# epifluidlab/FinaleToolkit

Hardware: AMD Instinct MI355X
Metric: genomic windows/sec (coverage+WPS+DELFI) at 30x WGS (higher is better)
Workload: dtype int32/int64

## Files before the change

finaletoolkit_amd/csrc/ftk_textparse.hip:

```cpp
#include <hip/hip_runtime.h>

#include <algorithm>

#include "ftk_textparse.h"

namespace ftk {
namespace {

constexpr int kT = 256;
constexpr int kB = 16;
static_assert(kT * kB == kTextBlockBytes, "block geometry");

struct Range {
    const uint8_t* text;
    size_t n;
    unsigned lead;
};
__device__ __forceinline__ Range range_of(const uint8_t* text, size_t n, const TextSummary* ind) {
    if (!ind) return {text, n, 0u};
    const unsigned off = ind->text_off, lead = off & 15u;
    return {text + (off - lead), ind->text_len ? (size_t)ind->text_len + lead : 0, lead};
}

__device__ __forceinline__ unsigned nl_mask16(const uint8_t* __restrict__ text, size_t off, size_t n, uint4& v) {
    unsigned m = 0;
    if (off + kB <= n) {
        v = *reinterpret_cast<const uint4*>(text + off);
    } else {
        unsigned w[4] = {0u, 0u, 0u, 0u};
        for (int j = 0; j < kB && off + j < n; ++j) w[j >> 2] |= (unsigned)text[off + j] << (8 * (j & 3));
        v = make_uint4(w[0], w[1], w[2], w[3]);
    }
    const unsigned w[4] = {v.x, v.y, v.z, v.w};
#pragma unroll
    for (int k = 0; k < 4; ++k)
#pragma unroll
        for (int j = 0; j < 4; ++j)
            if (((w[k] >> (8 * j)) & 0xffu) == (unsigned)'\n') m |= 1u << (4 * k + j);
    if (off + kB > n) m &= n > off ? (1u << (n - off)) - 1u : 0u;
    return m;
}

__device__ __forceinline__ unsigned wave_incl_scan(unsigned v, int lane) {
#pragma unroll
    for (int d = 1; d < 64; d <<= 1) {
        const unsigned t = __shfl_up(v, d, 64);
        if (lane >= d) v += t;
    }
    return v;
}

constexpr unsigned long long kAgg = 1ull << 32, kIncl = 2ull << 32;
__device__ __forceinline__ unsigned long long st_load(const unsigned long long* p) {
    return __hip_atomic_load(p, __ATOMIC_RELAXED, __HIP_MEMORY_SCOPE_AGENT);
}
__device__ __forceinline__ void st_store(unsigned long long* p, unsigned long long v) {
    __hip_atomic_store(p, v, __ATOMIC_RELAXED, __HIP_MEMORY_SCOPE_AGENT);
}

struct GlobalText {
    const uint8_t* __restrict__ p;
    __device__ __forceinline__ uint8_t operator[](uint32_t i) const { return p[i]; }
};
struct LdsText {
    const uint8_t* p;
    uint32_t base;
    __device__ __forceinline__ uint8_t operator[](uint32_t i) const { return p[i - base]; }
};

template <typename Text>
__device__ __forceinline__ bool dev_digits(const Text& t, uint32_t& p, uint32_t e, uint8_t term, unsigned long long& v) {
    const uint32_t s = p;
    unsigned long long x = 0;
    while (p < e) {
        const unsigned d = (unsigned)t[p] - (unsigned)'0';
        if (d > 9) break;
        x = x * 10 + d;
        ++p;
    }
    if (p == s || p - s > 10 || p >= e || t[p] != term) return false;
    ++p;
    v = x;
    return true;
}

template <typename Text>
__device__ __forceinline__ bool parse_row(const Text& t, size_t i, uint32_t b, uint32_t e, uint32_t pb, bool last,
                                          size_t max_lines, int bed6, int32_t* __restrict__ o_start, int32_t* __restrict__ o_end,
                                          uint8_t* __restrict__ o_mapq, uint8_t* __restrict__ o_strand,
                                          TextSummary* __restrict__ sum, int indirect) {
    uint32_t p = b;
    while (p < e && t[p] != '\t') ++p;
    const uint32_t name_len = p - b;
    unsigned long long fs = 0, fe = 0, mq = 0;
    uint8_t strand = 0;
    bool ok = name_len > 0 && p < e && t[b] != '#';
    if (ok) {
        ++p;
        ok = dev_digits(t, p, e, '\t', fs) && dev_digits(t, p, e, '\t', fe);
    }
    if (ok && bed6) {
        while (p < e && t[p] != '\t') ++p;
        ok = p < e;
        ++p;
    }
    if (ok) ok = dev_digits(t, p, e, '\t', mq);
    if (ok) {
        ok = p < e;
        if (ok) {
            strand = t[p];
            ok = strand != '\t' && strand != '\r';
            ++p;
            if (p < e && t[p] == '\r') ++p;
            ok = ok && p == e;
        }
    }
    ok = ok && fs <= 0x7fffffffull && fe <= 0x7fffffffull;
    if (ok && i < max_lines) {
        o_start[i] = (int32_t)fs;
        o_end[i] = (int32_t)fe;
        o_mapq[i] = (uint8_t)(mq < 255 ? mq : 255);
        o_strand[i] = strand == '+' ? 1 : 0;
        bool new_run = i == 0;
        if (!new_run) {
            const uint32_t pe = b - 1;
            new_run = pb + name_len >= pe || t[pb + name_len] != '\t';
            for (uint32_t k = 0; !new_run && k < name_len; ++k) new_run = t[pb + k] != t[b + k];
        }
        if (new_run) {
            const unsigned slot = atomicAdd(&sum->n_runs, 1u);
            if (slot < (unsigned)kTextMaxRuns) {
                sum->run_line[slot] = (unsigned)i;
                sum->run_off[slot] = b;
            }
            if (indirect) {
                if (slot < (unsigned)kTextNamedRuns && name_len < (uint32_t)kTextNameBytes) {
                    for (uint32_t k = 0; k < name_len; ++k) sum->run_name[slot][k] = t[b + k];
                    sum->run_name[slot][name_len] = 0;
                } else {
                    sum->name_overflow = 1;
                }
            }
        }
    }
    if (!ok && last) sum->last_line_bad = 1;
    return ok;
}

template <typename Text>
__device__ __forceinline__ uint32_t line_start_before(const Text& t, uint32_t from, uint32_t lead) {
    uint32_t p = from;
    while (p > lead && t[p - 1] != '\n') --p;
    return p;
}

constexpr int kHalo = 256;
constexpr int kMaxLinesPerBlock = 512;
__global__ __launch_bounds__(kT) void lines_rows_kernel(const uint8_t* __restrict__ text_, size_t n_,
                                                         unsigned long long* __restrict__ state, unsigned n_max_blocks,
                                                         size_t max_lines, int bed6, int32_t* __restrict__ o_start,
                                                         int32_t* __restrict__ o_end, uint8_t* __restrict__ o_mapq,
                                                         uint8_t* __restrict__ o_strand, TextSummary* __restrict__ sum,
                                                         int indirect) {
    __shared__ unsigned s_bid, s_base, s_first, s_prev;
    __shared__ unsigned wave_tot[kT / 64];
    __shared__ unsigned short nlpos[kMaxLinesPerBlock];
    __shared__ __align__(16) uint8_t s_text[kHalo + kTextBlockBytes];
    const int tid = threadIdx.x, lane = tid & 63, wv = tid >> 6;
    if (tid == 0) s_bid = atomicAdd(reinterpret_cast<unsigned*>(state + n_max_blocks), 1u);
    __syncthreads();
    const unsigned bid = s_bid;
    const Range R = range_of(text_, n_, indirect ? sum : nullptr);
    const uint8_t* __restrict__ text = R.text;
    const size_t n = R.n;
    const unsigned n_blocks = (unsigned)((n + kTextBlockBytes - 1) / kTextBlockBytes);
    if (bid >= n_blocks) {
        if (bid == 0 && tid == 0) sum->n_lines = 0;
        return;
    }
    const size_t blk_off = (size_t)bid * kTextBlockBytes;
    const size_t off = blk_off + (size_t)tid * kB;
    uint4 mine = make_uint4(0u, 0u, 0u, 0u);
    unsigned m = off < n ? nl_mask16(text, off, n, mine) : 0;
    *reinterpret_cast<uint4*>(&s_text[kHalo + tid * kB]) = mine;
    if (tid < kHalo / kB && bid > 0)
        *reinterpret_cast<uint4*>(&s_text[tid * kB]) = *reinterpret_cast<const uint4*>(text + blk_off - kHalo + (size_t)tid * kB);
    if (off == 0) m &= ~0u << R.lead;
    const unsigned c = __popc(m);
    const unsigned incl = wave_incl_scan(c, lane);
    if (lane == 63) wave_tot[wv] = incl;
    __syncthreads();
    unsigned before = 0, total = 0;
#pragma unroll
    for (int k = 0; k < kT / 64; ++k) {
        if (k < wv) before += wave_tot[k];
        total += wave_tot[k];
    }
    {
        unsigned idx = before + incl - c;
        while (m) {
            const int j = __ffs(m) - 1;
            m &= m - 1;
            if (idx < (unsigned)kMaxLinesPerBlock) nlpos[idx] = (unsigned short)(tid * kB + j);
            ++idx;
        }
    }
    if (wv == 0) {
        unsigned base = 0;
        if (bid > 0) {
            if (lane == 0) st_store(state + bid, kAgg | total);
            int j = (int)bid - 1;
            for (;;) {
                const int idx = j - lane;
                unsigned long long v = kIncl;
                if (idx >= 0)
                    do v = st_load(state + idx);
                    while ((v >> 32) == 0ull);
                const unsigned long long done = __ballot((v >> 32) == 2ull);
                const int stop = done ? __ffsll(done) - 1 : 63;
                unsigned part = lane <= stop ? (unsigned)v : 0u;
#pragma unroll
                for (int d = 32; d > 0; d >>= 1) part += __shfl_down(part, d, 64);
                base += (unsigned)__shfl(part, 0, 64);
                if (done) break;
                j -= 64;
            }
        }
        if (lane == 0) {
            st_store(state + bid, kIncl | (unsigned long long)(base + total));
            s_base = base;
            if (bid == n_blocks - 1) {
                sum->n_lines = (unsigned long long)base + total;
                if ((size_t)base + total > max_lines) sum->overflow = 1;
            }
        }
    }
    __syncthreads();
    if (total == 0) return;
    if (total > (unsigned)kMaxLinesPerBlock) {
        if (tid == 0) sum->overflow = 1;
        return;
    }
    const uint32_t lds_lo = bid > 0 ? (uint32_t)blk_off - (uint32_t)kHalo : 0u;
    const LdsText LT{s_text, (uint32_t)blk_off - (uint32_t)kHalo};
    const GlobalText GT{text};
    if (wv == 0) {
        const uint32_t e0 = (uint32_t)blk_off + nlpos[0];
        const uint32_t span = e0 - max(R.lead, lds_lo);
        const bool all_seen = lds_lo <= R.lead;
        const bool v0 = (uint32_t)lane < span, v1 = (uint32_t)lane + 64u < span;
        const unsigned long long m0 = __ballot(v0 && LT[e0 - 1u - (uint32_t)lane] == '\n');
        const unsigned long long m1 = __ballot(v1 && LT[e0 - 65u - (uint32_t)lane] == '\n');
        if (lane == 0) {
            const uint32_t seen = min(span, 128u);
            uint32_t f, pv;
            const int k1 = m0 ? __ffsll(m0) - 1 : (m1 ? 64 + __ffsll(m1) - 1 : -1);
            if (k1 >= 0) f = e0 - (uint32_t)k1;
            else f = (all_seen && span <= 128u) ? R.lead : line_start_before(GT, e0 - seen, R.lead);
            if (f == R.lead) {
                pv = f;
            } else {
                int k2 = -1;
                if (k1 >= 0) {
                    const unsigned long long r0 = k1 < 63 ? m0 & (~0ull << (k1 + 1)) : 0ull;
                    const unsigned long long r1 = k1 < 64 ? m1 : (k1 < 127 ? m1 & (~0ull << (k1 - 63)) : 0ull);
                    k2 = r0 ? __ffsll(r0) - 1 : (r1 ? 64 + __ffsll(r1) - 1 : -1);
                }
                if (k2 >= 0) pv = e0 - (uint32_t)k2;
                else if (k1 >= 0 && all_seen && span <= 128u) pv = R.lead;
                else pv = line_start_before(GT, k1 >= 0 ? e0 - seen : f - 1u, R.lead);
            }
            s_first = f;
            s_prev = pv;
        }
    }
    __syncthreads();
    const unsigned base = s_base;
    const uint32_t last_e = (uint32_t)(n - 1);
    for (unsigned k0 = 0; k0 < total; k0 += kT) {
        const unsigned k = k0 + (unsigned)tid;
        bool bad = false;
        if (k < total) {
            const uint32_t e = (uint32_t)blk_off + nlpos[k];
            const uint32_t b = k > 0 ? (uint32_t)blk_off + nlpos[k - 1] + 1u : s_first;
            const uint32_t pb = k > 1 ? (uint32_t)blk_off + nlpos[k - 2] + 1u : (k == 1 ? s_first : s_prev);
            const size_t i = (size_t)base + k;
            if (min(b, pb) >= lds_lo)
                bad = !parse_row(LT, i, b, e, pb, e == last_e, max_lines, bed6, o_start, o_end, o_mapq, o_strand, sum, indirect);
            else
                bad = !parse_row(GT, i, b, e, pb, e == last_e, max_lines, bed6, o_start, o_end, o_mapq, o_strand, sum, indirect);
        }
        const unsigned long long mask = __ballot(bad);
        if (lane == 0 && mask) atomicAdd(&sum->n_bad, (unsigned long long)__popcll(mask));
    }
}

__global__ __launch_bounds__(256) void piece_setup_kernel(uint8_t* __restrict__ text, uint32_t data_off, uint32_t data_len,
                                                          const uint8_t* __restrict__ prev_text,
                                                          const TextSummary* __restrict__ prev_sum, uint32_t first_skip,
                                                          int eof, TextSummary* __restrict__ sum,
                                                          unsigned long long* __restrict__ state, unsigned n_state) {
    __shared__ unsigned best;
    const int tid = threadIdx.x;
    if (blockIdx.x > 0) {
        for (size_t k = (size_t)(blockIdx.x - 1) * 256 + tid; k < n_state; k += (size_t)(gridDim.x - 1) * 256) state[k] = 0ull;
        return;
    }
    unsigned tail_prev = 0, prev_end = 0;
    if (prev_sum) {
        tail_prev = prev_sum->tail_len;
        prev_end = prev_sum->text_off + prev_sum->text_len;
    }
    if (tail_prev > kTextCarryMax || tail_prev > data_off) {
        if (tid == 0) sum->carry_overflow = 1;
        tail_prev = 0;
    }
    for (unsigned k = tid; k < tail_prev; k += 256) text[data_off - tail_prev + k] = prev_text[prev_end + k];
    const unsigned off = data_off - tail_prev + (prev_sum ? 0u : min(first_skip, data_len));
    unsigned end = data_off + data_len;
    if (tid == 0) best = 0;
    __syncthreads();
    const unsigned lo = end - off > kTextCarryMax ? end - kTextCarryMax : off;
    unsigned mine = 0;
    for (unsigned p = lo + tid; p < end; p += 256)
        if (text[p] == '\n') mine = p + 1;
    atomicMax(&best, mine);
    __syncthreads();
    if (tid == 0) {
        unsigned last = best;
        if (eof && end > off && last != end) {
            text[end] = '\n';
            last = ++end;
        }
        if (last == 0) {
            sum->text_off = off;
            sum->text_len = 0;
            sum->tail_len = end - off;
            if (end - off > kTextCarryMax) sum->carry_overflow = 1;
        } else {
            sum->text_off = off;
            sum->text_len = last - off;
            sum->tail_len = end - last;
        }
    }
}

template <bool BAM>
__global__ __launch_bounds__(256) void append_rows_kernel(int32_t* __restrict__ ds, int32_t* __restrict__ de,
                                                          uint8_t* __restrict__ dq, uint8_t* __restrict__ dt,
                                                          int32_t* __restrict__ da, int32_t* __restrict__ db,
                                                          const int32_t* __restrict__ ss, const int32_t* __restrict__ se,
                                                          const uint8_t* __restrict__ sq, const uint8_t* __restrict__ st,
                                                          const int32_t* __restrict__ sa, const int32_t* __restrict__ sb,
                                                          size_t n) {
    const size_t stride = (size_t)gridDim.x * blockDim.x;
    for (size_t i = (size_t)blockIdx.x * blockDim.x + threadIdx.x; i < n; i += stride) {
        ds[i] = __builtin_nontemporal_load(ss + i);
        de[i] = __builtin_nontemporal_load(se + i);
        dq[i] = __builtin_nontemporal_load(sq + i);
        dt[i] = __builtin_nontemporal_load(st + i);
        if (BAM) {
            da[i] = __builtin_nontemporal_load(sa + i);
            db[i] = __builtin_nontemporal_load(sb + i);
        }
    }
}

}

void append_rows_launch(hipStream_t s, int32_t* dst_start, int32_t* dst_end, uint8_t* dst_mapq, uint8_t* dst_strand,
                        int32_t* dst_r1s, int32_t* dst_r1e, const int32_t* src_start, const int32_t* src_end,
                        const uint8_t* src_mapq, const uint8_t* src_strand, const int32_t* src_r1s, const int32_t* src_r1e,
                        size_t n) {
    if (!n) return;
    const unsigned blocks = (unsigned)std::min<size_t>((n + 255) / 256, 4096);
    if (dst_r1s)
        hipLaunchKernelGGL(append_rows_kernel<true>, dim3(blocks), dim3(256), 0, s, dst_start, dst_end, dst_mapq, dst_strand,
                           dst_r1s, dst_r1e, src_start, src_end, src_mapq, src_strand, src_r1s, src_r1e, n);
    else
        hipLaunchKernelGGL(append_rows_kernel<false>, dim3(blocks), dim3(256), 0, s, dst_start, dst_end, dst_mapq, dst_strand,
                           dst_r1s, dst_r1e, src_start, src_end, src_mapq, src_strand, src_r1s, src_r1e, n);
}

size_t textparse_scratch_bytes(size_t text_bytes) {
    return ((text_bytes + kTextCarryMax + 64) / kTextBlockBytes + 4) * sizeof(unsigned long long);
}

void textparse_launch_inflated(hipStream_t s, uint8_t* d_text, uint32_t data_off, uint32_t data_len,
                               const uint8_t* prev_text, const TextSummary* prev_sum, uint32_t first_skip, bool eof, bool bed6,
                               void* d_scratch, size_t max_lines, int32_t* d_start, int32_t* d_end, uint8_t* d_mapq,
                               uint8_t* d_strand, TextSummary* d_sum) {
    const size_t n_max = (size_t)kTextCarryMax + data_len + 32;
    const unsigned n_blocks = (unsigned)((n_max + kTextBlockBytes - 1) / kTextBlockBytes);
    unsigned long long* state = static_cast<unsigned long long*>(d_scratch);
    const unsigned zero_blocks = std::min(64u, (n_blocks + 1 + 255) / 256);
    hipLaunchKernelGGL(piece_setup_kernel, dim3(1 + zero_blocks), dim3(256), 0, s, d_text, data_off, data_len, prev_text, prev_sum,
                       first_skip, eof ? 1 : 0, d_sum, state, n_blocks + 1);
    hipLaunchKernelGGL(lines_rows_kernel, dim3(n_blocks), dim3(kT), 0, s, d_text, (size_t)0, state, n_blocks, max_lines,
                       bed6 ? 1 : 0, d_start, d_end, d_mapq, d_strand, d_sum, 1);
}

void textparse_launch(hipStream_t s, const uint8_t* d_text, size_t n, bool bed6, void* d_scratch, size_t max_lines,
                      int32_t* d_start, int32_t* d_end, uint8_t* d_mapq, uint8_t* d_strand, TextSummary* d_sum) {
    if (n == 0) return;
    const unsigned n_blocks = (unsigned)((n + kTextBlockBytes - 1) / kTextBlockBytes);
    unsigned long long* state = static_cast<unsigned long long*>(d_scratch);
    (void)hipMemsetAsync(state, 0, ((size_t)n_blocks + 1) * sizeof(unsigned long long), s);
    hipLaunchKernelGGL(lines_rows_kernel, dim3(n_blocks), dim3(kT), 0, s, d_text, n, state, n_blocks, max_lines, bed6 ? 1 : 0,
                       d_start, d_end, d_mapq, d_strand, d_sum, 0);
}

}
```

Before: 6.797 million.

## Add SWAR word-level BED row parser and backward vectorized newline search

```diff
diff --git a/finaletoolkit_amd/csrc/ftk_textparse.hip b/finaletoolkit_amd/csrc/ftk_textparse.hip
--- a/finaletoolkit_amd/csrc/ftk_textparse.hip
+++ b/finaletoolkit_amd/csrc/ftk_textparse.hip
@@ -82,6 +82,33 @@
     ++p;
     v = x;
     return true;
+}
+
+template <typename Text>
+__device__ __forceinline__ void emit_row(const Text& t, size_t i, uint32_t b, uint32_t name_len, unsigned long long fs,
+                                         unsigned long long fe, unsigned long long mq, uint8_t strand, bool new_run,
+                                         int32_t* __restrict__ o_start, int32_t* __restrict__ o_end,
+                                         uint8_t* __restrict__ o_mapq, uint8_t* __restrict__ o_strand,
+                                         TextSummary* __restrict__ sum, int indirect) {
+    o_start[i] = (int32_t)fs;
+    o_end[i] = (int32_t)fe;
+    o_mapq[i] = (uint8_t)(mq < 255 ? mq : 255);
+    o_strand[i] = strand == '+' ? 1 : 0;
+    if (new_run) {
+        const unsigned slot = atomicAdd(&sum->n_runs, 1u);
+        if (slot < (unsigned)kTextMaxRuns) {
+            sum->run_line[slot] = (unsigned)i;
+            sum->run_off[slot] = b;
+        }
+        if (indirect) {
+            if (slot < (unsigned)kTextNamedRuns && name_len < (uint32_t)kTextNameBytes) {
+                for (uint32_t k = 0; k < name_len; ++k) sum->run_name[slot][k] = t[b + k];
+                sum->run_name[slot][name_len] = 0;
+            } else {
+                sum->name_overflow = 1;
+            }
+        }
+    }
 }
 
 template <typename Text>
@@ -117,34 +144,102 @@
     }
     ok = ok && fs <= 0x7fffffffull && fe <= 0x7fffffffull;
     if (ok && i < max_lines) {
-        o_start[i] = (int32_t)fs;
-        o_end[i] = (int32_t)fe;
-        o_mapq[i] = (uint8_t)(mq < 255 ? mq : 255);
-        o_strand[i] = strand == '+' ? 1 : 0;
         bool new_run = i == 0;
         if (!new_run) {
             const uint32_t pe = b - 1;
             new_run = pb + name_len >= pe || t[pb + name_len] != '\t';
             for (uint32_t k = 0; !new_run && k < name_len; ++k) new_run = t[pb + k] != t[b + k];
         }
-        if (new_run) {
-            const unsigned slot = atomicAdd(&sum->n_runs, 1u);
-            if (slot < (unsigned)kTextMaxRuns) {
-                sum->run_line[slot] = (unsigned)i;
-                sum->run_off[slot] = b;
-            }
-            if (indirect) {
-                if (slot < (unsigned)kTextNamedRuns && name_len < (uint32_t)kTextNameBytes) {
-                    for (uint32_t k = 0; k < name_len; ++k) sum->run_name[slot][k] = t[b + k];
-                    sum->run_name[slot][name_len] = 0;
-                } else {
-                    sum->name_overflow = 1;
-                }
-            }
-        }
+        emit_row(t, i, b, name_len, fs, fe, mq, strand, new_run, o_start, o_end, o_mapq, o_strand, sum, indirect);
     }
     if (!ok && last) sum->last_line_bad = 1;
     return ok;
+}
+
+constexpr unsigned long long kOnes = 0x0101010101010101ull, kHigh = 0x8080808080808080ull, kLow7 = 0x7f7f7f7f7f7f7f7full;
+constexpr int kWordLine = 64;
+
+__device__ __forceinline__ unsigned long long eq_bytes(unsigned long long x, uint8_t c) {
+    const unsigned long long y = x ^ (kOnes * c);
+    return ~(((y & kLow7) + kLow7) | y | kLow7);
+}
+__device__ __forceinline__ unsigned long long digit_bytes(unsigned long long x) {
+    const unsigned long long ge0 = (x | kHigh) - kOnes * 0x30u;
+    const unsigned long long gt9 = (x & kLow7) + kOnes * 0x46u;
+    return ge0 & ~gt9 & ~x & kHigh;
+}
+__device__ __forceinline__ unsigned flag_bits(unsigned long long f) { return (unsigned)(((f >> 7) * 0x0102040810204080ull) >> 56); }
+__device__ __forceinline__ unsigned long long low_bits(unsigned n) { return n >= 64 ? ~0ull : (1ull << n) - 1ull; }
+
+struct LdsWords {
+    const unsigned long long* w;
+    unsigned last;
+    __device__ __forceinline__ unsigned long long at(uint32_t idx) const {
+        const unsigned a = min(idx >> 3, last), sh = (idx & 7u) * 8u;
+        const unsigned long long lo = w[a], hi = w[min(a + 1u, last)];
+        return sh ? (lo >> sh) | (hi << (64u - sh)) : lo;
+    }
+};
+
+__device__ __forceinline__ bool word_digits(unsigned long long x0, unsigned long long x1, unsigned len, unsigned long long& v) {
+    const unsigned n0 = min(len, 8u);
+    const unsigned long long f0 = kHigh & low_bits(8u * n0), f1 = len > 8u ? kHigh & low_bits(8u * (len - 8u)) : 0ull;
+    if ((digit_bytes(x0) & f0) != f0 || (digit_bytes(x1) & f1) != f1) return false;
+    unsigned long long d = n0 < 8u ? x0 << (64u - 8u * n0) : x0;
+    d = ((d & 0x0f0f0f0f0f0f0f0full) * 2561ull) >> 8;
+    d = ((d & 0x00ff00ff00ff00ffull) * 6553601ull) >> 16;
+    d = ((d & 0x0000ffff0000ffffull) * 42949672960001ull) >> 32;
+    if (len > 8u) {
+        const unsigned d8 = (unsigned)(x1 & 15u), d9 = (unsigned)((x1 >> 8) & 15u);
+        d = len == 9u ? d * 10u + d8 : d * 100u + d8 * 10u + d9;
+    }
+    v = d;
+    return true;
+}
+
+__device__ __forceinline__ bool word_row(const uint8_t* s_text, const LdsWords& W, uint32_t bi, uint32_t ei, unsigned& name_len,
+                                         unsigned long long& fs, unsigned long long& fe, unsigned long long& mq,
+                                         uint8_t& strand) {
+    const uint32_t a = bi & ~15u;
+    if (ei - a >= (uint32_t)kWordLine) return false;
+    const uint32_t top = ei & ~15u;
+    unsigned long long tabs = 0;
+#pragma unroll
+    for (int k = 0; k < kWordLine / 16; ++k) {
+        const uint4 q = *reinterpret_cast<const uint4*>(s_text + min(a + 16u * k, top));
+        const unsigned long long lo = (unsigned long long)q.y << 32 | q.x, hi = (unsigned long long)q.w << 32 | q.z;
+        tabs |= (unsigned long long)(flag_bits(eq_bytes(lo, '\t')) | flag_bits(eq_bytes(hi, '\t')) << 8) << (16 * k);
+    }
+    const unsigned br = bi - a, er = ei - a;
+    tabs &= low_bits(er) & ~low_bits(br);
+    if (__popcll(tabs) != 4) return false;
+    const unsigned t1 = __ffsll(tabs) - 1;
+    tabs &= tabs - 1;
+    const unsigned t2 = __ffsll(tabs) - 1;
+    tabs &= tabs - 1;
+    const unsigned t3 = __ffsll(tabs) - 1;
+    tabs &= tabs - 1;
+    const unsigned t4 = __ffsll(tabs) - 1;
+    name_len = t1 - br;
+    if (name_len == 0 || name_len >= (unsigned)kTextNameBytes || er - t4 < 2u || er - t4 > 3u) return false;
+    const unsigned long long tail = W.at(a + t4 + 1u), head = W.at(bi);
+    strand = (uint8_t)tail;
+    if (strand == '\r' || (er - t4 == 3u && (uint8_t)(tail >> 8) != '\r') || (uint8_t)head == '#') return false;
+    const unsigned l1 = t2 - t1 - 1u, l2 = t3 - t2 - 1u, l3 = t4 - t3 - 1u;
+    if (l1 - 1u > 9u || l2 - 1u > 9u || l3 - 1u > 9u) return false;
+    const bool ok = word_digits(W.at(a + t1 + 1u), W.at(a + t1 + 9u), l1, fs) &&
+                    word_digits(W.at(a + t2 + 1u), W.at(a + t2 + 9u), l2, fe) &&
+                    word_digits(W.at(a + t3 + 1u), W.at(a + t3 + 9u), l3, mq);
+    return ok && fs <= 0x7fffffffull && fe <= 0x7fffffffull;
+}
+
+__device__ __forceinline__ bool words_equal(const LdsWords& W, uint32_t pb, uint32_t b, unsigned n) {
+    bool eq = true;
+    for (unsigned k = 0; eq && k < n; k += 8u) {
+        const unsigned long long m = low_bits(8u * (n - k));
+        eq = ((W.at(pb + k) ^ W.at(b + k)) & m) == 0ull;
+    }
+    return eq;
 }
 
 template <typename Text>
@@ -156,7 +251,8 @@
 
 constexpr int kHalo = 256;
 constexpr int kMaxLinesPerBlock = 512;
-__global__ __launch_bounds__(kT) void lines_rows_kernel(const uint8_t* __restrict__ text_, size_t n_,
+__global__ __launch_bounds__(kT) __attribute__((amdgpu_waves_per_eu(8, 8)))
+void lines_rows_kernel(const uint8_t* __restrict__ text_, size_t n_,
                                                          unsigned long long* __restrict__ state, unsigned n_max_blocks,
                                                          size_t max_lines, int bed6, int32_t* __restrict__ o_start,
                                                          int32_t* __restrict__ o_end, uint8_t* __restrict__ o_mapq,
@@ -244,6 +340,7 @@
     const uint32_t lds_lo = bid > 0 ? (uint32_t)blk_off - (uint32_t)kHalo : 0u;
     const LdsText LT{s_text, (uint32_t)blk_off - (uint32_t)kHalo};
     const GlobalText GT{text};
+    const LdsWords LW{reinterpret_cast<const unsigned long long*>(s_text), (unsigned)(kHalo + kTextBlockBytes) / 8u - 1u};
     if (wv == 0) {
         const uint32_t e0 = (uint32_t)blk_off + nlpos[0];
         const uint32_t span = e0 - max(R.lead, lds_lo);
@@ -285,10 +382,21 @@
             const uint32_t b = k > 0 ? (uint32_t)blk_off + nlpos[k - 1] + 1u : s_first;
             const uint32_t pb = k > 1 ? (uint32_t)blk_off + nlpos[k - 2] + 1u : (k == 1 ? s_first : s_prev);
             const size_t i = (size_t)base + k;
-            if (min(b, pb) >= lds_lo)
+            const bool in_lds = min(b, pb) >= lds_lo;
+            unsigned name_len;
+            unsigned long long fs, fe, mq;
+            uint8_t strand;
+            if (in_lds && !bed6 && word_row(s_text, LW, b - LT.base, e - LT.base, name_len, fs, fe, mq, strand)) {
+                if (i < max_lines) {
+                    const bool new_run = i == 0 || pb + name_len >= b - 1u ||
+                                         !words_equal(LW, pb - LT.base, b - LT.base, name_len + 1u);
+                    emit_row(LT, i, b, name_len, fs, fe, mq, strand, new_run, o_start, o_end, o_mapq, o_strand, sum, indirect);
+                }
+            } else if (in_lds) {
                 bad = !parse_row(LT, i, b, e, pb, e == last_e, max_lines, bed6, o_start, o_end, o_mapq, o_strand, sum, indirect);
-            else
+            } else {
                 bad = !parse_row(GT, i, b, e, pb, e == last_e, max_lines, bed6, o_start, o_end, o_mapq, o_strand, sum, indirect);
+            }
         }
         const unsigned long long mask = __ballot(bad);
         if (lane == 0 && mask) atomicAdd(&sum->n_bad, (unsigned long long)__popcll(mask));
@@ -321,10 +429,27 @@
     if (tid == 0) best = 0;
     __syncthreads();
     const unsigned lo = end - off > kTextCarryMax ? end - kTextCarryMax : off;
-    unsigned mine = 0;
-    for (unsigned p = lo + tid; p < end; p += 256)
-        if (text[p] == '\n') mine = p + 1;
-    atomicMax(&best, mine);
+    if (end > lo) {
+        const unsigned first = lo & ~15u;
+        for (unsigned top = ((end - 1u) & ~15u) + 16u; top > first; top = top - first > 4096u ? top - 4096u : first) {
+            unsigned mine = 0;
+            const unsigned q = top - 16u * (unsigned)(tid + 1);
+            if (top - first >= 16u * (unsigned)(tid + 1)) {
+                const uint4 v = *reinterpret_cast<const uint4*>(text + q);
+                const unsigned w[4] = {v.x, v.y, v.z, v.w};
+#pragma unroll
+                for (int j = 0; j < 16; ++j) {
+                    const unsigned p = q + (unsigned)j;
+                    if (((w[j >> 2] >> (8 * (j & 3))) & 0xffu) == (unsigned)'\n' && p >= lo && p < end) mine = p + 1;
+                }
+            }
+            if (mine) atomicMax(&best, mine);
+            __syncthreads();
+            const unsigned found = best;
+            __syncthreads();
+            if (found) break;
+        }
+    }
     __syncthreads();
     if (tid == 0) {
         unsigned last = best;
```

Result: no change. 6.806 million (median of 4 runs) (+0.1%).
